# dohlee/rosettafold-pytorch

Hardware: AMD Instinct MI355X
Metric: residues/sec forward (L=256, N=128) (higher is better)
Workload: dtype bf16; 1 GPU; BASELINE.json configs[1]: bsz=4/GPU, n_seq=128, L=256, d_msa=384, d_pair=288, 8+5 blocks, 4 encoder layers, random-init weights; global_batch=4, parallelism=batch-sharded x1 (replicated weights), launch=one hipGraph replay per step (validation + input copy outside the graph)

## Files before the change

rosettafold-pytorch_amd/csrc/favor.hip:

```cpp
#include <type_traits>

#include "common.h"

#define FV_DH 64
#define FV_M 266
#define FV_MT 17
#define FV_MPAD 288
#define FV_CTX_LD 592
#define FV_DT 5
#define FV_DROWS 80

struct FavorAttnP {
  const h16_t* qkv;
  const h16_t* pc;
  h16_t* out;
  int64_t x_b, x_o, x_s;
  int64_t x_h;
  int64_t o_b, o_o, o_s;
  int q_off, k_off, v_off;
  int n_o, n_h, nitems;
  int nchunks;
  int dbg;
  float eps;
  float ctx_scale;
  int seq_len;
};

#ifdef RF_H16_IS_F16
#define FV_CS(x) ((x) * p.ctx_scale)
#else
#define FV_CS(x) (x)
#endif

typedef __attribute__((ext_vector_type(4))) short s16x4;

__device__ __forceinline__ int swz_off(int row, int chunk) { return row * 128 + ((chunk ^ (row & 7)) << 4); }

template <bool TAIL = false>
__device__ __forceinline__ void fv_load_tile(char* smem, int lds_off, const h16_t* g, int64_t stride, int nrows,
                                             int wave, int lane, int nvalid = 0) {
  const int ninstr = nrows * 8 / 64;
  for (int it = wave; it < ninstr; it += 4) {
    const int slot = it * 64 + lane;
    const int row = slot >> 3;
    const int clog = (slot & 7) ^ (row & 7);
    const int srow = TAIL ? (row < nvalid ? row : nvalid - 1) : row;
    rf_glds16(g + (int64_t)srow * stride + clog * 8, smem + lds_off + it * 1024);
  }
}

__device__ __forceinline__ float rbf(float x) { return h2f(f2h(x)); }

__device__ __forceinline__ float fv_mfma_done(float acc_reg) {
  asm volatile("s_nop 7\n\ts_nop 3" : "+v"(acc_reg));
  return acc_reg;
}

union Frag {
  h16x8 v;
  unsigned u[4];
  uint2 h[2];
};

template <int LS, bool SOFTMAX, bool TAIL>
__global__ __launch_bounds__(256, 1) void favor_attention_kernel(const FavorAttnP p) {
  constexpr int ST = LS / 64;
  constexpr int NSB = LS / 32;
  constexpr int PC_OFF = 0;
  constexpr int K_OFF = FV_MPAD * 128;
  constexpr int V_OFF = K_OFF + LS * 128;
  constexpr int CTX_OFF = V_OFF + LS * 128;
  constexpr int DIAG_OFF = CTX_OFF + FV_DROWS * FV_CTX_LD;
  constexpr int RED_OFF = DIAG_OFF + LS * 4;
  extern __shared__ __attribute__((aligned(16))) char smem[];
  const int tid = threadIdx.x, lane = tid & 63;
  const int wave = __builtin_amdgcn_readfirstlane(tid >> 6) & 3;
  const int fr = lane & 15, fq = lane >> 4;
  const int nm = wave == 0 ? 5 : 4;
  const int m0t = wave == 0 ? 0 : 5 + 4 * (wave - 1);
  const f32x4 epsv = {p.eps, p.eps, p.eps, p.eps};
  Frag ones;
#pragma unroll
  for (int k = 0; k < 4; ++k) ones.u[k] = fr == 0 ? RF_H16_ONE2 : 0u;

  fv_load_tile(smem, PC_OFF, p.pc, FV_DH, FV_MPAD, wave, lane);
  for (int i = tid; i < FV_DROWS * FV_CTX_LD / 4; i += 256) ((unsigned*)(smem + CTX_OFF))[i] = 0u;

  auto item_base = [&](int item, int64_t& xb, int64_t& ob) {
    const int h = item % p.n_h;
    const int t = item / p.n_h;
    const int o = t % p.n_o, b = t / p.n_o;
    xb = (int64_t)b * p.x_b + (int64_t)o * p.x_o + (int64_t)h * p.x_h;
    ob = (int64_t)b * p.o_b + (int64_t)o * p.o_o + h * FV_DH;
  };

  const int nch = p.nchunks;
  const int nv = TAIL ? p.seq_len : 0;
  int item = blockIdx.x;
  if (item < p.nitems) {
    int64_t xb, ob;
    item_base(item, xb, ob);
    fv_load_tile<TAIL>(smem, K_OFF, p.qkv + xb + p.k_off, p.x_s, LS, wave, lane, nv);
    fv_load_tile<TAIL>(smem, V_OFF, p.qkv + xb + p.v_off, p.x_s, LS, wave, lane, nv);
  }
  bool first = true;
  for (; item < p.nitems; item += gridDim.x) {
    int64_t xb, ob;
    item_base(item, xb, ob);
    if (first || TAIL)
      asm volatile("s_waitcnt vmcnt(0)" ::: "memory");
    else
      asm volatile("s_waitcnt vmcnt(%0)" ::"n"(ST * 4) : "memory");
    first = false;
    __syncthreads();
    h16x8 qf[ST][2];
    auto load_q = [&](int chunk) {
#pragma unroll
      for (int t = 0; t < ST; ++t) {
        int s = chunk * LS + (wave * ST + t) * 16 + fr;
        if (TAIL) s = s < nv ? s : nv - 1;
        const h16_t* qrow = p.qkv + xb + p.q_off + (int64_t)s * p.x_s;
#pragma unroll
        for (int kk = 0; kk < 2; ++kk) qf[t][kk] = *(const h16x8*)(qrow + (kk * 4 + fq) * 8);
      }
    };
    load_q(0);

    float gmax = 0.f;
    if constexpr (SOFTMAX) {
      for (int s = tid; s < LS; s += 256) {
        float a = 0.f;
#pragma unroll
        for (int c = 0; c < 8; ++c) {
          const h16x8 x = *(const h16x8*)(smem + K_OFF + s * 128 + c * 16);
#pragma unroll
          for (int e = 0; e < 8; ++e) {
            const float f = h2f((h16_t)x[e]);
            a = fmaf(f, f, a);
          }
        }
        ((float*)(smem + DIAG_OFF))[s] = a * (0.0625f * 1.4426950408889634f);
      }
    }

    h16x8 pf[5][2];
#pragma unroll
    for (int j = 0; j < 5; ++j)
#pragma unroll
      for (int kk = 0; kk < 2; ++kk)
        if (j < nm) pf[j][kk] = *(const h16x8*)(smem + PC_OFF + swz_off((m0t + j) * 16 + fr, kk * 4 + fq));

    if constexpr (SOFTMAX) {
      float mx = -INFINITY;
      const int nsb0 = TAIL ? (nv + 31) >> 5 : NSB;
      for (int u = 0; u < nsb0; ++u) {
        h16x8 kf[2][2];
#pragma unroll
        for (int t = 0; t < 2; ++t)
#pragma unroll
          for (int kk = 0; kk < 2; ++kk)
            kf[t][kk] = *(const h16x8*)(smem + K_OFF + swz_off((2 * u + t) * 16 + fr, kk * 4 + fq));
#pragma unroll
        for (int j = 0; j < 5; ++j) {
          if (j < nm) {
            const bool valid = (m0t + j) * 16 + fr < FV_M;
#pragma unroll
            for (int t = 0; t < 2; ++t) {
              f32x4 a = {0.f, 0.f, 0.f, 0.f};
              a = rf_mfma16(kf[t][0], pf[j][0], a, 0, 0, 0);
              a = rf_mfma16(kf[t][1], pf[j][1], a, 0, 0, 0);
              if (valid) mx = fmaxf(mx, fmaxf(fmaxf(a[0], a[1]), fmaxf(a[2], a[3])));
            }
          }
        }
      }
      mx = wave_max(mx);
      if (lane == 0) ((float*)(smem + RED_OFF))[wave] = mx;
      __syncthreads();
      const float* red = (const float*)(smem + RED_OFF);
      gmax = fmaxf(fmaxf(red[0], red[1]), fmaxf(red[2], red[3]));
    }

    f32x4 ctx[5][FV_DT];
#pragma unroll
    for (int j = 0; j < 5; ++j)
#pragma unroll
      for (int i = 0; i < FV_DT; ++i) ctx[j][i] = (f32x4){0.f, 0.f, 0.f, 0.f};
    for (int ck = 0; ck < nch; ++ck) {
    const int rem = TAIL ? nv - ck * LS : LS;
    if (ck > 0) {
      __syncthreads();
      fv_load_tile<TAIL>(smem, K_OFF, p.qkv + xb + p.k_off + (int64_t)ck * LS * p.x_s, p.x_s, LS, wave, lane, rem);
      fv_load_tile<TAIL>(smem, V_OFF, p.qkv + xb + p.v_off + (int64_t)ck * LS * p.x_s, p.x_s, LS, wave, lane, rem);
      asm volatile("s_waitcnt vmcnt(0)" ::: "memory");
      __syncthreads();
    }
    const int nsb = TAIL ? (rem < LS ? (rem + 31) >> 5 : NSB) : NSB;
    for (int u = 0; u < nsb; ++u) {
      h16x8 kf[2][2];
#pragma unroll
      for (int t = 0; t < 2; ++t)
#pragma unroll
        for (int kk = 0; kk < 2; ++kk)
          kf[t][kk] = *(const h16x8*)(smem + K_OFF + swz_off((2 * u + t) * 16 + fr, kk * 4 + fq));
      Frag vf[4];
      {
        const int p4 = fr & 3;
#pragma unroll
        for (int i = 0; i < 4; ++i) {
#pragma unroll
          for (int half = 0; half < 2; ++half) {
            const int row = u * 32 + half * 16 + 4 * fq + (fr >> 2);
            const int off = V_OFF + swz_off(row, i * 2 + (p4 >> 1)) + (p4 & 1) * 8;
            const s16x4 r = __builtin_amdgcn_ds_read_tr16_b64_v4i16((__attribute__((address_space(3))) s16x4*)(smem + off));
            vf[i].h[half] = __builtin_bit_cast(uint2, r);
          }
        }
      }
      f32x4 init[2] = {epsv, epsv};
      if constexpr (SOFTMAX) {
#pragma unroll
        for (int t = 0; t < 2; ++t) {
          const float4 d4 = *(const float4*)(smem + DIAG_OFF + ((2 * u + t) * 16 + 4 * fq) * 4);
          init[t] = (f32x4){-(d4.x + gmax), -(d4.y + gmax), -(d4.z + gmax), -(d4.w + gmax)};
        }
      }
#pragma unroll
      for (int j = 0; j < 5; ++j) {
        if (j < nm) {
          f32x4 a[2];
#pragma unroll
          for (int t = 0; t < 2; ++t) {
            a[t] = rf_mfma16(kf[t][0], pf[j][0], init[t], 0, 0, 0);
            a[t] = rf_mfma16(kf[t][1], pf[j][1], a[t], 0, 0, 0);
          }
          float f[2][4];
#pragma unroll
          for (int t = 0; t < 2; ++t)
#pragma unroll
            for (int r = 0; r < 4; ++r) {
              if constexpr (SOFTMAX)
                f[t][r] = __builtin_amdgcn_exp2f(a[t][r]) + p.eps;
              else
                f[t][r] = fmaxf(a[t][r], p.eps);
            }
          if ((m0t + j) == FV_MT - 1 && fr >= FV_M - 16 * (FV_MT - 1)) {
#pragma unroll
            for (int t = 0; t < 2; ++t)
#pragma unroll
              for (int r = 0; r < 4; ++r) f[t][r] = 0.f;
          }
          if constexpr (TAIL) {
            if ((u + 1) * 32 > rem) {
#pragma unroll
              for (int t = 0; t < 2; ++t)
#pragma unroll
                for (int r = 0; r < 4; ++r) f[t][r] = (2 * u + t) * 16 + 4 * fq + r < rem ? f[t][r] : 0.f;
            }
          }
          Frag kfr;
          kfr.u[0] = rf_pack2_h16(f[0][0], f[0][1]);
          kfr.u[1] = rf_pack2_h16(f[0][2], f[0][3]);
          kfr.u[2] = rf_pack2_h16(f[1][0], f[1][1]);
          kfr.u[3] = rf_pack2_h16(f[1][2], f[1][3]);
#pragma unroll
          for (int i = 0; i < 4; ++i)
            ctx[j][i] = rf_mfma16(kfr.v, vf[i].v, ctx[j][i], 0, 0, 0);
          ctx[j][4] = rf_mfma16(kfr.v, ones.v, ctx[j][4], 0, 0, 0);
        }
      }
    }
    }
#pragma unroll
    for (int j = 0; j < 5; ++j) {
      if (j < nm) {
#pragma unroll
        for (int i = 0; i < FV_DT; ++i) {
          uint2 w;
          w.x = rf_pack2_h16(FV_CS(ctx[j][i][0]), FV_CS(ctx[j][i][1]));
          w.y = rf_pack2_h16(FV_CS(ctx[j][i][2]), FV_CS(ctx[j][i][3]));
          *(uint2*)(smem + CTX_OFF + (i * 16 + fr) * FV_CTX_LD + ((m0t + j) * 16 + 4 * fq) * 2) = w;
        }
      }
    }
    __syncthreads();

    asm volatile("s_waitcnt vmcnt(0)" ::: "memory");
    {
      const int nxt = item + gridDim.x;
      if (nxt < p.nitems) {
        int64_t xb2, ob2;
        item_base(nxt, xb2, ob2);
        fv_load_tile<TAIL>(smem, K_OFF, p.qkv + xb2 + p.k_off, p.x_s, LS, wave, lane, nv);
        fv_load_tile<TAIL>(smem, V_OFF, p.qkv + xb2 + p.v_off, p.x_s, LS, wave, lane, nv);
      }
    }

    f32x4 qinit[ST];
#pragma unroll
    for (int t = 0; t < ST; ++t) qinit[t] = epsv;
    if constexpr (SOFTMAX) {
      float dq[ST], rmax[ST];
#pragma unroll
      for (int t = 0; t < ST; ++t) {
        float a = 0.f;
#pragma unroll
        for (int kk = 0; kk < 2; ++kk)
#pragma unroll
          for (int e = 0; e < 8; ++e) {
            const float f = h2f((h16_t)qf[t][kk][e]);
            a = fmaf(f, f, a);
          }
        a += __shfl_xor(a, 16, 64);
        a += __shfl_xor(a, 32, 64);
        dq[t] = a * (0.0625f * 1.4426950408889634f);
        rmax[t] = -INFINITY;
      }
      for (int j = 0; j < FV_MT; ++j) {
        h16x8 pfr[2];
#pragma unroll
        for (int kk = 0; kk < 2; ++kk) pfr[kk] = *(const h16x8*)(smem + PC_OFF + swz_off(j * 16 + fr, kk * 4 + fq));
#pragma unroll
        for (int t = 0; t < ST; ++t) {
          f32x4 a = {0.f, 0.f, 0.f, 0.f};
          a = rf_mfma16(pfr[0], qf[t][0], a, 0, 0, 0);
          a = rf_mfma16(pfr[1], qf[t][1], a, 0, 0, 0);
#pragma unroll
          for (int r = 0; r < 4; ++r)
            if (j * 16 + 4 * fq + r < FV_M) rmax[t] = fmaxf(rmax[t], a[r]);
        }
      }
#pragma unroll
      for (int t = 0; t < ST; ++t) {
        rmax[t] = fmaxf(rmax[t], __shfl_xor(rmax[t], 16, 64));
        rmax[t] = fmaxf(rmax[t], __shfl_xor(rmax[t], 32, 64));
        const float off = -(dq[t] + rmax[t]);
        qinit[t] = (f32x4){off, off, off, off};
      }
    }
    for (int qc = 0; qc < nch; ++qc) {
    if (TAIL && qc * LS + wave * ST * 16 >= nv) continue;
    if (qc > 0) load_q(qc);
    f32x4 num[FV_DT][ST];
#pragma unroll
    for (int t = 0; t < ST; ++t)
#pragma unroll
      for (int i = 0; i < FV_DT; ++i) num[i][t] = (f32x4){0.f, 0.f, 0.f, 0.f};
    auto mblock = [&](int u, auto last_tag) {
      constexpr bool LAST = decltype(last_tag)::value;
      float f[2][ST][4];
#pragma unroll
      for (int jj = 0; jj < 2; ++jj) {
        if (LAST && jj == 1) {
#pragma unroll
          for (int t = 0; t < ST; ++t)
#pragma unroll
            for (int r = 0; r < 4; ++r) f[jj][t][r] = 0.f;
        } else {
          const int j = 2 * u + jj;
          h16x8 pfr[2];
#pragma unroll
          for (int kk = 0; kk < 2; ++kk) pfr[kk] = *(const h16x8*)(smem + PC_OFF + swz_off(j * 16 + fr, kk * 4 + fq));
#pragma unroll
          for (int t = 0; t < ST; ++t) {
            f32x4 a = rf_mfma16(pfr[0], qf[t][0], qinit[t], 0, 0, 0);
            a = rf_mfma16(pfr[1], qf[t][1], a, 0, 0, 0);
#pragma unroll
            for (int r = 0; r < 4; ++r) {
              float x;
              if constexpr (SOFTMAX)
                x = __builtin_amdgcn_exp2f(a[r]) + p.eps;
              else
                x = fmaxf(a[r], p.eps);
              if (LAST && 4 * fq + r >= FV_M - 16 * (FV_MT - 1)) x = 0.f;
              f[jj][t][r] = x;
            }
          }
        }
      }
      Frag cf[FV_DT];
#pragma unroll
      for (int i = 0; i < FV_DT; ++i) {
        const char* base = smem + CTX_OFF + (i * 16 + fr) * FV_CTX_LD + (32 * u + 4 * fq) * 2;
        cf[i].h[0] = *(const uint2*)base;
        cf[i].h[1] = *(const uint2*)(base + 32);
      }
#pragma unroll
      for (int t = 0; t < ST; ++t) {
        Frag qfr;
        qfr.u[0] = rf_pack2_h16(f[0][t][0], f[0][t][1]);
        qfr.u[1] = rf_pack2_h16(f[0][t][2], f[0][t][3]);
        qfr.u[2] = rf_pack2_h16(f[1][t][0], f[1][t][1]);
        qfr.u[3] = rf_pack2_h16(f[1][t][2], f[1][t][3]);
#pragma unroll
        for (int i = 0; i < FV_DT; ++i)
          num[i][t] = rf_mfma16(cf[i].v, qfr.v, num[i][t], 0, 0, 0);
      }
    };
    for (int u = 0; u < (FV_MT - 1) / 2; ++u) mblock(u, std::false_type{});
    mblock((FV_MT - 1) / 2, std::true_type{});
#pragma unroll
    for (int t = 0; t < ST; ++t) {
      const float dn = __shfl(fv_mfma_done(num[4][t][0]), fr, 64);
      const float inv = 1.f / dn;
      const int s = qc * LS + (wave * ST + t) * 16 + fr;
      h16_t* orow = p.out + ob + (int64_t)s * p.o_s;
#pragma unroll
      for (int i = 0; i < 4; ++i) {
        uint2 w;
        w.x = rf_pack2_h16(num[i][t][0] * inv, num[i][t][1] * inv);
        w.y = rf_pack2_h16(num[i][t][2] * inv, num[i][t][3] * inv);
        if (!TAIL || s < nv) *(uint2*)(orow + i * 16 + 4 * fq) = w;
      }
    }
    }
  }
}

#pragma clang diagnostic ignored "-Winline-asm"
__device__ __forceinline__ void fv_glds_asm(const void* src, unsigned lds_addr) {
  asm volatile("s_mov_b32 m0, %0\n\ts_nop 0\n\tglobal_load_lds_dwordx4 %1, off" ::"s"(lds_addr), "v"(src) : "memory", "m0");
}

__device__ __forceinline__ void fv_lds_barrier() {
  asm volatile("s_waitcnt lgkmcnt(0)" ::: "memory");
  __builtin_amdgcn_s_barrier();
  asm volatile("" ::: "memory");
}

__device__ unsigned long long g_fv_cycles[8];
#define FV_STAMP(slot)                                                   \
  if (prof) {                                                            \
    const unsigned long long now = __builtin_readcyclecounter();         \
    acc_cyc[slot] += now - t_last;                                       \
    t_last = now;                                                        \
  }

template <int LS, bool SOFTMAX, bool TAIL>
__global__ __launch_bounds__(512, 1) void favor_attention_kernel8(const FavorAttnP p) {
  constexpr int NSB = LS / 32;
  constexpr int NJ = 3;
  constexpr int STB = LS >= 128 ? LS / 128 : 1;
  constexpr int NWB = LS / (16 * STB);
  constexpr int PC_OFF = 0;
  constexpr int K_OFF = FV_MPAD * 128;
  constexpr int V_OFF = K_OFF + LS * 128;
  constexpr int CTX_OFF = V_OFF + LS * 128;
  constexpr int DIAG_OFF = CTX_OFF + FV_DROWS * FV_CTX_LD;
  constexpr int RED_OFF = DIAG_OFF + LS * 4;
  extern __shared__ __attribute__((aligned(16))) char smem[];
  const int tid = threadIdx.x, lane = tid & 63;
  const int wave = __builtin_amdgcn_readfirstlane(tid >> 6) & 7;
  const int fr = lane & 15, fq = lane >> 4;
  const int nm = wave == 0 ? 3 : 2;
  const int m0t = wave == 0 ? 0 : 1 + 2 * wave;
  const f32x4 epsv = {p.eps, p.eps, p.eps, p.eps};
  Frag ones;
#pragma unroll
  for (int k = 0; k < 4; ++k) ones.u[k] = fr == 0 ? RF_H16_ONE2 : 0u;

  const unsigned lds_base = (unsigned)(uintptr_t)(__attribute__((address_space(3))) char*)smem;
  auto load_tile8 = [&](int lds_off, const h16_t* gp, int64_t stride, auto nrows_tag, int nvalid = 0) {
    constexpr int NI = decltype(nrows_tag)::value * 8 / 64;
    int ln = lane;
    asm volatile("" : "+v"(ln));
    const int dma_row = ln >> 3;
    const int dma_col = ((ln & 7) ^ dma_row) * 8;
    const h16_t* g0 = gp + (int64_t)dma_row * stride + dma_col;
#pragma unroll
    for (int k = 0; k < (NI + 7) / 8; ++k) {
      const int it = wave + 8 * k;
      if (NI % 8 == 0 || it < NI) {
        const unsigned dst = __builtin_amdgcn_readfirstlane(lds_base + lds_off + it * 1024);
        if (TAIL && nvalid > 0) {
          const int row = dma_row + 8 * it;
          fv_glds_asm(gp + (int64_t)(row < nvalid ? row : nvalid - 1) * stride + dma_col, dst);
        } else {
          fv_glds_asm(g0 + (int64_t)(8 * it) * stride, dst);
        }
      }
    }
  };
  constexpr std::integral_constant<int, LS> LS_TAG{};
  load_tile8(PC_OFF, p.pc, FV_DH, std::integral_constant<int, FV_MPAD>{});
  for (int i = tid; i < FV_DROWS * FV_CTX_LD / 4; i += 512) ((unsigned*)(smem + CTX_OFF))[i] = 0u;

  auto item_base = [&](int item, int64_t& xb, int64_t& ob) {
    const int h = item % p.n_h;
    const int t = item / p.n_h;
    const int o = t % p.n_o, b = t / p.n_o;
    xb = (int64_t)b * p.x_b + (int64_t)o * p.x_o + (int64_t)h * p.x_h;
    ob = (int64_t)b * p.o_b + (int64_t)o * p.o_o + h * FV_DH;
  };
  auto ctx_col = [](int tile, int q4) { return ((tile >> 1) * 32 + 8 * q4 + 4 * (tile & 1)) * 2; };
  const int nch = SOFTMAX ? 1 : p.nchunks;
  const int nv = TAIL ? p.seq_len : 0;
  int item = blockIdx.x;
  if (item < p.nitems) {
    int64_t xb, ob;
    item_base(item, xb, ob);
    load_tile8(K_OFF, p.qkv + xb + p.k_off, p.x_s, LS_TAG, nv);
    load_tile8(V_OFF, p.qkv + xb + p.v_off, p.x_s, LS_TAG, nv);
  }
  bool first = true;
  const bool prof = (RF_DBG(p.dbg) & 8) && wave == ((RF_DBG(p.dbg) >> 4) & 7);
  unsigned long long acc_cyc[7] = {0, 0, 0, 0, 0, 0, 0};
  unsigned long long t_last = prof ? __builtin_readcyclecounter() : 0;
  for (; item < p.nitems; item += gridDim.x) {
    int64_t xb, ob;
    item_base(item, xb, ob);
    asm volatile("" : "+v"(xb), "+v"(ob));
    if (prof) {
      t_last = __builtin_readcyclecounter();
      acc_cyc[6] += 1;
    }
    if (first || wave >= NWB || TAIL)
      asm volatile("s_waitcnt vmcnt(0)" ::: "memory");
    else
      asm volatile("s_waitcnt vmcnt(%0)" ::"n"(STB * 4) : "memory");
    first = false;
    fv_lds_barrier();
    FV_STAMP(0)
    h16x8 pf[NJ][2];
    {
      int frP = fr, fqP = fq;
      asm volatile("" : "+v"(frP), "+v"(fqP));
#pragma unroll
      for (int j = 0; j < NJ; ++j)
#pragma unroll
        for (int kk = 0; kk < 2; ++kk)
          pf[j][kk] = *(const h16x8*)(smem + PC_OFF + m0t * 2048 + swz_off(frP, kk * 4 + fqP) + (j < nm ? j : 0) * 2048);
    }
    h16x8 qf[STB][2];
    auto load_q = [&](int chunk) {
      int frq = fr, fqq = fq;
      asm volatile("" : "+v"(frq), "+v"(fqq));
      if (wave < NWB) {
#pragma unroll
        for (int t = 0; t < STB; ++t) {
          int s = chunk * LS + (wave * STB + t) * 16 + frq;
          if (TAIL) s = s < nv ? s : nv - 1;
          const h16_t* qrow = p.qkv + xb + p.q_off + (int64_t)s * p.x_s;
#pragma unroll
          for (int kk = 0; kk < 2; ++kk) qf[t][kk] = *(const h16x8*)(qrow + (kk * 4 + fqq) * 8);
        }
      }
    };
    load_q(0);

    float gmax = 0.f;
    if constexpr (SOFTMAX) {
      int frS = fr, fqS = fq;
      asm volatile("" : "+v"(frS), "+v"(fqS));
      for (int s = tid; s < LS; s += 512) {
        float a = 0.f;
#pragma unroll
        for (int c = 0; c < 8; ++c) {
          const h16x8 x = *(const h16x8*)(smem + K_OFF + s * 128 + c * 16);
#pragma unroll
          for (int e = 0; e < 8; ++e) {
            const float f = h2f((h16_t)x[e]);
            a = fmaf(f, f, a);
          }
        }
        ((float*)(smem + DIAG_OFF))[s] = a * (0.0625f * 1.4426950408889634f);
      }
      float mx = -INFINITY;
      const int nsb0 = TAIL ? (nv + 31) >> 5 : NSB;
      for (int u = 0; u < nsb0; ++u) {
        h16x8 kf[2][2];
#pragma unroll
        for (int t = 0; t < 2; ++t)
#pragma unroll
          for (int kk = 0; kk < 2; ++kk)
            kf[t][kk] = *(const h16x8*)(smem + K_OFF + swz_off((2 * u + t) * 16 + frS, kk * 4 + fqS));
#pragma unroll
        for (int j = 0; j < NJ; ++j) {
          if (j < nm) {
            const h16x8* pfj = pf[j];
            const bool valid = (m0t + j) != FV_MT - 1 || frS < FV_M - 16 * (FV_MT - 1);
#pragma unroll
            for (int t = 0; t < 2; ++t) {
              f32x4 a = {0.f, 0.f, 0.f, 0.f};
              a = rf_mfma16(kf[t][0], pfj[0], a, 0, 0, 0);
              a = rf_mfma16(kf[t][1], pfj[1], a, 0, 0, 0);
              if (valid) mx = fmaxf(mx, fmaxf(fmaxf(a[0], a[1]), fmaxf(a[2], a[3])));
            }
          }
        }
      }
      mx = wave_max(mx);
      if (lane == 0) ((float*)(smem + RED_OFF))[wave] = mx;
      fv_lds_barrier();
      const float* red = (const float*)(smem + RED_OFF);
      gmax = fmaxf(fmaxf(fmaxf(red[0], red[1]), fmaxf(red[2], red[3])), fmaxf(fmaxf(red[4], red[5]), fmaxf(red[6], red[7])));
    }

    f32x4 ctx[NJ][FV_DT];
#pragma unroll
    for (int j = 0; j < NJ; ++j)
#pragma unroll
      for (int i = 0; i < FV_DT; ++i) ctx[j][i] = (f32x4){0.f, 0.f, 0.f, 0.f};
    for (int ck = 0; ck < nch; ++ck) {
      const int rem = TAIL ? nv - ck * LS : LS;
      if (ck > 0) {
        __syncthreads();
        load_tile8(K_OFF, p.qkv + xb + p.k_off + (int64_t)ck * LS * p.x_s, p.x_s, LS_TAG, rem);
        load_tile8(V_OFF, p.qkv + xb + p.v_off + (int64_t)ck * LS * p.x_s, p.x_s, LS_TAG, rem);
        asm volatile("s_waitcnt vmcnt(0)" ::: "memory");
        __syncthreads();
      }
      const int nsb = TAIL ? (rem < LS ? (rem + 31) >> 5 : NSB) : NSB;
      h16x8 kf[2][2];
      Frag vf[4];
      auto load_sblock = [&](int u, h16x8 (&kfo)[2][2], Frag (&vfo)[4]) {
#pragma unroll
        for (int t = 0; t < 2; ++t)
#pragma unroll
          for (int kk = 0; kk < 2; ++kk)
            kfo[t][kk] = *(const h16x8*)(smem + K_OFF + swz_off((2 * u + t) * 16 + fr, kk * 4 + fq));
        const int p4 = fr & 3;
#pragma unroll
        for (int i = 0; i < 4; ++i) {
#pragma unroll
          for (int half = 0; half < 2; ++half) {
            const int row = u * 32 + half * 16 + 4 * fq + (fr >> 2);
            const int off = V_OFF + swz_off(row, i * 2 + (p4 >> 1)) + (p4 & 1) * 8;
            const s16x4 r = __builtin_amdgcn_ds_read_tr16_b64_v4i16((__attribute__((address_space(3))) s16x4*)(smem + off));
            vfo[i].h[half] = __builtin_bit_cast(uint2, r);
          }
        }
      };
      load_sblock(0, kf, vf);
      for (int u = 0; u < ((RF_DBG(p.dbg) & 1) ? 0 : nsb); ++u) {
        h16x8 kfn[2][2];
        Frag vfn[4];
        load_sblock(u + 1 < nsb ? u + 1 : u, kfn, vfn);
        f32x4 init[2] = {epsv, epsv};
        if constexpr (SOFTMAX) {
#pragma unroll
          for (int t = 0; t < 2; ++t) {
            const float4 d4 = *(const float4*)(smem + DIAG_OFF + ((2 * u + t) * 16 + 4 * fq) * 4);
            init[t] = (f32x4){-(d4.x + gmax), -(d4.y + gmax), -(d4.z + gmax), -(d4.w + gmax)};
          }
        }
#pragma unroll
        for (int j = 0; j < NJ; ++j) {
          if (j < nm) {
            const h16x8* pfj = pf[j];
            f32x4 a[2];
#pragma unroll
            for (int t = 0; t < 2; ++t) {
              a[t] = rf_mfma16(kf[t][0], pfj[0], init[t], 0, 0, 0);
              a[t] = rf_mfma16(kf[t][1], pfj[1], a[t], 0, 0, 0);
            }
            float f[2][4];
#pragma unroll
            for (int t = 0; t < 2; ++t)
#pragma unroll
              for (int r = 0; r < 4; ++r) {
                if constexpr (SOFTMAX)
                  f[t][r] = __builtin_amdgcn_exp2f(a[t][r]) + p.eps;
                else
                  f[t][r] = fmaxf(a[t][r], p.eps);
              }
            if ((m0t + j) == FV_MT - 1 && fr >= FV_M - 16 * (FV_MT - 1)) {
#pragma unroll
              for (int t = 0; t < 2; ++t)
#pragma unroll
                for (int r = 0; r < 4; ++r) f[t][r] = 0.f;
            }
            if constexpr (TAIL) {
              if ((u + 1) * 32 > rem) {
#pragma unroll
                for (int t = 0; t < 2; ++t)
#pragma unroll
                  for (int r = 0; r < 4; ++r) f[t][r] = (2 * u + t) * 16 + 4 * fq + r < rem ? f[t][r] : 0.f;
              }
            }
            Frag kfr;
            kfr.u[0] = rf_pack2_h16(f[0][0], f[0][1]);
            kfr.u[1] = rf_pack2_h16(f[0][2], f[0][3]);
            kfr.u[2] = rf_pack2_h16(f[1][0], f[1][1]);
            kfr.u[3] = rf_pack2_h16(f[1][2], f[1][3]);
#pragma unroll
            for (int i = 0; i < 4; ++i)
              ctx[j][i] = rf_mfma16(kfr.v, vf[i].v, ctx[j][i], 0, 0, 0);
            ctx[j][4] = rf_mfma16(kfr.v, ones.v, ctx[j][4], 0, 0, 0);
          }
        }
#pragma unroll
        for (int t = 0; t < 2; ++t)
#pragma unroll
          for (int kk = 0; kk < 2; ++kk) kf[t][kk] = kfn[t][kk];
#pragma unroll
        for (int i = 0; i < 4; ++i) vf[i] = vfn[i];
      }
    }
    FV_STAMP(1)
#pragma unroll
    for (int j = 0; j < NJ; ++j)
      if (j < nm) {
#pragma unroll
        for (int i = 0; i < FV_DT; ++i) {
          uint2 w;
          w.x = rf_pack2_h16(FV_CS(ctx[j][i][0]), FV_CS(ctx[j][i][1]));
          w.y = rf_pack2_h16(FV_CS(ctx[j][i][2]), FV_CS(ctx[j][i][3]));
          *(uint2*)(smem + CTX_OFF + (i * 16 + fr) * FV_CTX_LD + ctx_col(m0t + j, fq)) = w;
        }
      }
    fv_lds_barrier();
    FV_STAMP(2)
    asm volatile("s_waitcnt vmcnt(0)" ::: "memory");
#pragma unroll
    for (int t = 0; t < STB; ++t) {
      asm volatile("" : "+v"(qf[t][0]), "+v"(qf[t][1]));
    }
    {
      const int nxt = item + gridDim.x;
      if (nxt < p.nitems) {
        int64_t xb2, ob2;
        item_base(nxt, xb2, ob2);
        load_tile8(K_OFF, p.qkv + xb2 + p.k_off, p.x_s, LS_TAG, nv);
        load_tile8(V_OFF, p.qkv + xb2 + p.v_off, p.x_s, LS_TAG, nv);
      }
    }
    FV_STAMP(3)
    for (int qc = 0; qc < nch; ++qc) {
      if (qc > 0) {
        load_q(qc);
        asm volatile("s_waitcnt vmcnt(0)" ::: "memory");
#pragma unroll
        for (int t = 0; t < STB; ++t) {
          asm volatile("" : "+v"(qf[t][0]), "+v"(qf[t][1]));
        }
      }
      if (wave < NWB && (!TAIL || qc * LS + wave * STB * 16 < nv)) {
        f32x4 qinit[STB];
#pragma unroll
        for (int t = 0; t < STB; ++t) qinit[t] = epsv;
        if constexpr (SOFTMAX) {
          float dq[STB], rmax[STB];
#pragma unroll
          for (int t = 0; t < STB; ++t) {
            float a = 0.f;
#pragma unroll
            for (int kk = 0; kk < 2; ++kk)
#pragma unroll
              for (int e = 0; e < 8; ++e) {
                const float f = h2f((h16_t)qf[t][kk][e]);
                a = fmaf(f, f, a);
              }
            a += __shfl_xor(a, 16, 64);
            a += __shfl_xor(a, 32, 64);
            dq[t] = a * (0.0625f * 1.4426950408889634f);
            rmax[t] = -INFINITY;
          }
          for (int j = 0; j < FV_MT; ++j) {
            h16x8 pfr[2];
#pragma unroll
            for (int kk = 0; kk < 2; ++kk) pfr[kk] = *(const h16x8*)(smem + PC_OFF + swz_off(j * 16 + fr, kk * 4 + fq));
#pragma unroll
            for (int t = 0; t < STB; ++t) {
              f32x4 a = {0.f, 0.f, 0.f, 0.f};
              a = rf_mfma16(pfr[0], qf[t][0], a, 0, 0, 0);
              a = rf_mfma16(pfr[1], qf[t][1], a, 0, 0, 0);
#pragma unroll
              for (int r = 0; r < 4; ++r)
                if (j * 16 + 4 * fq + r < FV_M) rmax[t] = fmaxf(rmax[t], a[r]);
            }
          }
#pragma unroll
          for (int t = 0; t < STB; ++t) {
            rmax[t] = fmaxf(rmax[t], __shfl_xor(rmax[t], 16, 64));
            rmax[t] = fmaxf(rmax[t], __shfl_xor(rmax[t], 32, 64));
            const float off = -(dq[t] + rmax[t]);
            qinit[t] = (f32x4){off, off, off, off};
          }
        }
        f32x4 num[FV_DT][STB];
#pragma unroll
        for (int t = 0; t < STB; ++t)
#pragma unroll
          for (int i = 0; i < FV_DT; ++i) num[i][t] = (f32x4){0.f, 0.f, 0.f, 0.f};
        auto mblock = [&](int u, auto last_tag) {
          constexpr bool LAST = decltype(last_tag)::value;
          float f[2][STB][4];
#pragma unroll
          for (int jj = 0; jj < 2; ++jj) {
            if (LAST && jj == 1) {
#pragma unroll
              for (int t = 0; t < STB; ++t)
#pragma unroll
                for (int r = 0; r < 4; ++r) f[jj][t][r] = 0.f;
            } else {
              const int j = 2 * u + jj;
              h16x8 pfr[2];
#pragma unroll
              for (int kk = 0; kk < 2; ++kk) pfr[kk] = *(const h16x8*)(smem + PC_OFF + swz_off(j * 16 + fr, kk * 4 + fq));
#pragma unroll
              for (int t = 0; t < STB; ++t) {
                f32x4 a = rf_mfma16(pfr[0], qf[t][0], qinit[t], 0, 0, 0);
                a = rf_mfma16(pfr[1], qf[t][1], a, 0, 0, 0);
#pragma unroll
                for (int r = 0; r < 4; ++r) {
                  float x;
                  if constexpr (SOFTMAX)
                    x = __builtin_amdgcn_exp2f(a[r]) + p.eps;
                  else
                    x = fmaxf(a[r], p.eps);
                  if (LAST && 4 * fq + r >= FV_M - 16 * (FV_MT - 1)) x = 0.f;
                  f[jj][t][r] = x;
                }
              }
            }
          }
          Frag cf[FV_DT];
#pragma unroll
          for (int i = 0; i < FV_DT; ++i)
            cf[i].v = *(const h16x8*)(smem + CTX_OFF + (i * 16 + fr) * FV_CTX_LD + (32 * u + 8 * fq) * 2);
#pragma unroll
          for (int t = 0; t < STB; ++t) {
            Frag qfr;
            qfr.u[0] = rf_pack2_h16(f[0][t][0], f[0][t][1]);
            qfr.u[1] = rf_pack2_h16(f[0][t][2], f[0][t][3]);
            qfr.u[2] = rf_pack2_h16(f[1][t][0], f[1][t][1]);
            qfr.u[3] = rf_pack2_h16(f[1][t][2], f[1][t][3]);
#pragma unroll
            for (int i = 0; i < FV_DT; ++i)
              num[i][t] = rf_mfma16(cf[i].v, qfr.v, num[i][t], 0, 0, 0);
          }
        };
        for (int u = 0; u < ((RF_DBG(p.dbg) & 2) ? 0 : (FV_MT - 1) / 2); ++u) mblock(u, std::false_type{});
        mblock((FV_MT - 1) / 2, std::true_type{});
        FV_STAMP(4)
#pragma unroll
        for (int t = 0; t < STB; ++t) {
          const float dn = __shfl(fv_mfma_done(num[4][t][0]), fr, 64);
          const float inv = 1.f / dn;
          const int s = qc * LS + (wave * STB + t) * 16 + fr;
          h16_t* orow = p.out + ob + (int64_t)s * p.o_s;
#pragma unroll
          for (int i = 0; i < 4; ++i) {
            uint2 w;
            w.x = rf_pack2_h16(num[i][t][0] * inv, num[i][t][1] * inv);
            w.y = rf_pack2_h16(num[i][t][2] * inv, num[i][t][3] * inv);
            if (!TAIL || s < nv) *(uint2*)(orow + i * 16 + 4 * fq) = w;
          }
        }
      }
    }
    FV_STAMP(5)
  }
  if (prof && lane == 0) {
#pragma unroll
    for (int i = 0; i < 7; ++i) atomicAdd(&g_fv_cycles[i], acc_cyc[i]);
  }
}

extern "C" int rf_favor_phase_cycles(unsigned long long* out7, int reset) {
  unsigned long long z[8] = {0, 0, 0, 0, 0, 0, 0, 0};
  if (out7 && hipMemcpyFromSymbol(out7, HIP_SYMBOL(g_fv_cycles), 7 * sizeof(unsigned long long)) != hipSuccess) return 1000 + (int)hipGetLastError();
  if (reset && hipMemcpyToSymbol(HIP_SYMBOL(g_fv_cycles), z, sizeof(z)) != hipSuccess) return 1000 + (int)hipGetLastError();
  return 0;
}

template <int LS, bool SM, bool TAIL>
static int launch_favor(const FavorAttnP& p, hipStream_t s) {
  const size_t lds = (size_t)FV_MPAD * 128 + 2 * (size_t)LS * 128 + (size_t)FV_DROWS * FV_CTX_LD + LS * 4 + 64;
  const int ncu = rf_num_cus() > 0 ? rf_num_cus() : 256;
  const int grid = p.nitems < ncu ? p.nitems : ncu;
  static const bool force4 = getenv("RF_FAVOR4") != nullptr;
  constexpr bool only4 = SM && LS > 128;
  if (only4 || force4) {
    auto k = favor_attention_kernel<LS, SM, TAIL>;
    if (const int e = rf_enable_big_lds<favor_attention_kernel<LS, SM, TAIL>>()) return e;
    hipLaunchKernelGGL(k, dim3(grid), dim3(256), lds, s, p);
  } else if constexpr (!only4) {
    auto k = favor_attention_kernel8<LS, SM, TAIL>;
    if (const int e = rf_enable_big_lds<favor_attention_kernel8<LS, SM, TAIL>>()) return e;
    hipLaunchKernelGGL(k, dim3(grid), dim3(512), lds, s, p);
  }
  return rf_launch_status();
}

extern "C" int rf_favor_attention(const void* qkv, const void* pc, void* out, const int64_t x_strides[4],
                                  const int64_t o_strides[3], int q_off, int k_off, int v_off, int n_b, int n_o,
                                  int n_h, int seq_len, int dim_head, int n_features, int softmax_kernel, float eps,
                                  void* stream) {
  if (dim_head != FV_DH || n_features != FV_M) return RF_EINVAL;
  if (seq_len < 1) return RF_EINVAL;
  int nchunks = 1, ls = seq_len <= 64 ? 64 : seq_len <= 128 ? 128 : 256;
  if (seq_len > 256) {
    if (softmax_kernel) return RF_EINVAL;
    nchunks = (seq_len + 255) / 256;
  }
  const bool tail = seq_len != nchunks * ls;
  if (((uintptr_t)qkv % 16) || ((uintptr_t)pc % 16) || ((uintptr_t)out % 8)) return RF_EALIGN;
  for (int i = 0; i < 3; ++i)
    if (x_strides[i] % 8 || o_strides[i] % 4) return RF_EALIGN;
  if (x_strides[3] % 8) return RF_EALIGN;
  if (q_off % 8 || k_off % 8 || v_off % 8) return RF_EALIGN;
  FavorAttnP p;
  p.qkv = (const h16_t*)qkv;
  p.pc = (const h16_t*)pc;
  p.out = (h16_t*)out;
  p.x_b = x_strides[0]; p.x_o = x_strides[1]; p.x_s = x_strides[2]; p.x_h = x_strides[3];
  p.o_b = o_strides[0]; p.o_o = o_strides[1]; p.o_s = o_strides[2];
  p.q_off = q_off; p.k_off = k_off; p.v_off = v_off;
  p.n_o = n_o; p.n_h = n_h;
  p.nitems = n_b * n_o * n_h;
  p.eps = eps;
  p.nchunks = nchunks;
  p.seq_len = seq_len;
  p.ctx_scale = 1.0f;
#ifdef RF_H16_IS_F16
  for (int n = 1; n < seq_len; n <<= 1) p.ctx_scale *= 0.5f;
#endif
  static int dbg = 0;
  static const int dbg_rc = rf_dbg_env("RF_FAVOR_DBG", &dbg);
  if (dbg_rc) return dbg_rc;
  p.dbg = dbg;
  hipStream_t s = (hipStream_t)stream;
#define FV_LAUNCH(LS_) \
  (tail ? (softmax_kernel ? launch_favor<LS_, true, true>(p, s) : launch_favor<LS_, false, true>(p, s)) \
        : (softmax_kernel ? launch_favor<LS_, true, false>(p, s) : launch_favor<LS_, false, false>(p, s)))
  if (ls == 256) return FV_LAUNCH(256);
  if (ls == 128) return FV_LAUNCH(128);
  return FV_LAUNCH(64);
#undef FV_LAUNCH
}
```

Baseline: 3126 residues/s.

## Cache softmax FAVOR feature logits in registers to skip recomputing MFMAs

In the softmax FAVOR attention path, the key-side and query-side projection logits computed during the max pass are now kept in registers (kl, ql). The second pass reuses them instead of re-running the MFMAs and reloading the projection and key fragments from LDS. Loops are fully unrolled so the register arrays stay statically indexed. Tail masking moves to a packed bitmask on the bf16 fragments. The cost is much higher register pressure, which may cause spills, plus a static_assert limiting the softmax form to LS<=128.

```diff
diff --git a/rosettafold-pytorch_amd/csrc/favor.hip b/rosettafold-pytorch_amd/csrc/favor.hip
--- a/rosettafold-pytorch_amd/csrc/favor.hip
+++ b/rosettafold-pytorch_amd/csrc/favor.hip
@@ -442,6 +442,7 @@
   constexpr int NJ = 3;
   constexpr int STB = LS >= 128 ? LS / 128 : 1;
   constexpr int NWB = LS / (16 * STB);
+  static_assert(!SOFTMAX || LS <= 128, "the softmax form keeps LS / 16 key-logit tiles per feature tile and STB = 1 query tiles");
   constexpr int PC_OFF = 0;
   constexpr int K_OFF = FV_MPAD * 128;
   constexpr int V_OFF = K_OFF + LS * 128;
@@ -461,6 +462,7 @@
 
   const unsigned lds_base = (unsigned)(uintptr_t)(__attribute__((address_space(3))) char*)smem;
   auto load_tile8 = [&](int lds_off, const h16_t* gp, int64_t stride, auto nrows_tag, int nvalid = 0) {
+    constexpr bool CLAMP = TAIL && decltype(nrows_tag)::value == LS;
     constexpr int NI = decltype(nrows_tag)::value * 8 / 64;
     int ln = lane;
     asm volatile("" : "+v"(ln));
@@ -472,7 +474,7 @@
       const int it = wave + 8 * k;
       if (NI % 8 == 0 || it < NI) {
         const unsigned dst = __builtin_amdgcn_readfirstlane(lds_base + lds_off + it * 1024);
-        if (TAIL && nvalid > 0) {
+        if constexpr (CLAMP) {
           const int row = dma_row + 8 * it;
           fv_glds_asm(gp + (int64_t)(row < nvalid ? row : nvalid - 1) * stride + dma_col, dst);
         } else {
@@ -514,10 +516,11 @@
       t_last = __builtin_readcyclecounter();
       acc_cyc[6] += 1;
     }
-    if (first || wave >= NWB || TAIL)
+    if (first || wave >= NWB || TAIL) {
       asm volatile("s_waitcnt vmcnt(0)" ::: "memory");
-    else
+    } else {
       asm volatile("s_waitcnt vmcnt(%0)" ::"n"(STB * 4) : "memory");
+    }
     first = false;
     fv_lds_barrier();
     FV_STAMP(0)
@@ -549,6 +552,7 @@
     load_q(0);
 
     float gmax = 0.f;
+    f32x4 kl[SOFTMAX ? NJ : 1][SOFTMAX ? 2 * NSB : 1];
     if constexpr (SOFTMAX) {
       int frS = fr, fqS = fq;
       asm volatile("" : "+v"(frS), "+v"(fqS));
@@ -566,25 +570,30 @@
         ((float*)(smem + DIAG_OFF))[s] = a * (0.0625f * 1.4426950408889634f);
       }
       float mx = -INFINITY;
-      const int nsb0 = TAIL ? (nv + 31) >> 5 : NSB;
-      for (int u = 0; u < nsb0; ++u) {
-        h16x8 kf[2][2];
-#pragma unroll
-        for (int t = 0; t < 2; ++t)
-#pragma unroll
-          for (int kk = 0; kk < 2; ++kk)
-            kf[t][kk] = *(const h16x8*)(smem + K_OFF + swz_off((2 * u + t) * 16 + frS, kk * 4 + fqS));
-#pragma unroll
-        for (int j = 0; j < NJ; ++j) {
-          if (j < nm) {
-            const h16x8* pfj = pf[j];
-            const bool valid = (m0t + j) != FV_MT - 1 || frS < FV_M - 16 * (FV_MT - 1);
-#pragma unroll
-            for (int t = 0; t < 2; ++t) {
-              f32x4 a = {0.f, 0.f, 0.f, 0.f};
-              a = rf_mfma16(kf[t][0], pfj[0], a, 0, 0, 0);
-              a = rf_mfma16(kf[t][1], pfj[1], a, 0, 0, 0);
-              if (valid) mx = fmaxf(mx, fmaxf(fmaxf(a[0], a[1]), fmaxf(a[2], a[3])));
+      int nsb0 = TAIL ? (nv + 31) >> 5 : NSB;
+      if constexpr (TAIL) asm volatile("" : "+s"(nsb0));
+#pragma unroll
+      for (int u = 0; u < NSB; ++u) {
+        if (!TAIL || u < nsb0) {
+          h16x8 kf[2][2];
+#pragma unroll
+          for (int t = 0; t < 2; ++t)
+#pragma unroll
+            for (int kk = 0; kk < 2; ++kk)
+              kf[t][kk] = *(const h16x8*)(smem + K_OFF + swz_off((2 * u + t) * 16 + frS, kk * 4 + fqS));
+#pragma unroll
+          for (int j = 0; j < NJ; ++j) {
+            if (j < nm) {
+              const h16x8* pfj = pf[j];
+              const bool valid = (m0t + j) != FV_MT - 1 || frS < FV_M - 16 * (FV_MT - 1);
+#pragma unroll
+              for (int t = 0; t < 2; ++t) {
+                f32x4 a = {0.f, 0.f, 0.f, 0.f};
+                a = rf_mfma16(kf[t][0], pfj[0], a, 0, 0, 0);
+                a = rf_mfma16(kf[t][1], pfj[1], a, 0, 0, 0);
+                kl[j][2 * u + t] = a;
+                if (valid) mx = fmaxf(mx, fmaxf(fmaxf(a[0], a[1]), fmaxf(a[2], a[3])));
+              }
             }
           }
         }
@@ -596,6 +605,8 @@
       gmax = fmaxf(fmaxf(fmaxf(red[0], red[1]), fmaxf(red[2], red[3])), fmaxf(fmaxf(red[4], red[5]), fmaxf(red[6], red[7])));
     }
 
+    int frA = fr, fqA = fq;
+    if constexpr (SOFTMAX) asm volatile("" : "+v"(frA), "+v"(fqA));
     f32x4 ctx[NJ][FV_DT];
 #pragma unroll
     for (int j = 0; j < NJ; ++j)
@@ -610,21 +621,24 @@
         asm volatile("s_waitcnt vmcnt(0)" ::: "memory");
         __syncthreads();
       }
-      const int nsb = TAIL ? (rem < LS ? (rem + 31) >> 5 : NSB) : NSB;
+      int nsb = TAIL ? (rem < LS ? (rem + 31) >> 5 : NSB) : NSB;
+      if constexpr (TAIL && SOFTMAX) asm volatile("" : "+s"(nsb));
       h16x8 kf[2][2];
       Frag vf[4];
       auto load_sblock = [&](int u, h16x8 (&kfo)[2][2], Frag (&vfo)[4]) {
-#pragma unroll
-        for (int t = 0; t < 2; ++t)
-#pragma unroll
-          for (int kk = 0; kk < 2; ++kk)
-            kfo[t][kk] = *(const h16x8*)(smem + K_OFF + swz_off((2 * u + t) * 16 + fr, kk * 4 + fq));
-        const int p4 = fr & 3;
+        if constexpr (!SOFTMAX) {
+#pragma unroll
+          for (int t = 0; t < 2; ++t)
+#pragma unroll
+            for (int kk = 0; kk < 2; ++kk)
+              kfo[t][kk] = *(const h16x8*)(smem + K_OFF + swz_off((2 * u + t) * 16 + frA, kk * 4 + fqA));
+        }
+        const int p4 = frA & 3;
 #pragma unroll
         for (int i = 0; i < 4; ++i) {
 #pragma unroll
           for (int half = 0; half < 2; ++half) {
-            const int row = u * 32 + half * 16 + 4 * fq + (fr >> 2);
+            const int row = u * 32 + half * 16 + 4 * fqA + (frA >> 2);
             const int off = V_OFF + swz_off(row, i * 2 + (p4 >> 1)) + (p4 & 1) * 8;
             const s16x4 r = __builtin_amdgcn_ds_read_tr16_b64_v4i16((__attribute__((address_space(3))) s16x4*)(smem + off));
             vfo[i].h[half] = __builtin_bit_cast(uint2, r);
@@ -632,27 +646,42 @@
         }
       };
       load_sblock(0, kf, vf);
-      for (int u = 0; u < ((RF_DBG(p.dbg) & 1) ? 0 : nsb); ++u) {
+      auto sblock = [&](const int u) {
         h16x8 kfn[2][2];
         Frag vfn[4];
-        load_sblock(u + 1 < nsb ? u + 1 : u, kfn, vfn);
+        load_sblock(SOFTMAX ? (u + 1 < NSB ? u + 1 : u) : (u + 1 < nsb ? u + 1 : u), kfn, vfn);
         f32x4 init[2] = {epsv, epsv};
         if constexpr (SOFTMAX) {
 #pragma unroll
           for (int t = 0; t < 2; ++t) {
-            const float4 d4 = *(const float4*)(smem + DIAG_OFF + ((2 * u + t) * 16 + 4 * fq) * 4);
+            const float4 d4 = *(const float4*)(smem + DIAG_OFF + ((2 * u + t) * 16 + 4 * fqA) * 4);
             init[t] = (f32x4){-(d4.x + gmax), -(d4.y + gmax), -(d4.z + gmax), -(d4.w + gmax)};
+          }
+        }
+        unsigned mk[4] = {~0u, ~0u, ~0u, ~0u};
+        if constexpr (SOFTMAX && TAIL) {
+          int left = rem - 4 * fqA;
+          asm volatile("" : "+v"(left));
+#pragma unroll
+          for (int i = 0; i < 4; ++i) {
+            const int r0 = (2 * u + (i >> 1)) * 16 + 2 * (i & 1);
+            mk[i] = ((unsigned)((r0 - left) >> 31) & 0xFFFFu) | ((unsigned)((r0 + 1 - left) >> 31) & 0xFFFF0000u);
           }
         }
 #pragma unroll
         for (int j = 0; j < NJ; ++j) {
           if (j < nm) {
-            const h16x8* pfj = pf[j];
             f32x4 a[2];
-#pragma unroll
-            for (int t = 0; t < 2; ++t) {
-              a[t] = rf_mfma16(kf[t][0], pfj[0], init[t], 0, 0, 0);
-              a[t] = rf_mfma16(kf[t][1], pfj[1], a[t], 0, 0, 0);
+            if constexpr (SOFTMAX) {
+#pragma unroll
+              for (int t = 0; t < 2; ++t) a[t] = kl[j][2 * u + t] + init[t];
+            } else {
+              const h16x8* pfj = pf[j];
+#pragma unroll
+              for (int t = 0; t < 2; ++t) {
+                a[t] = rf_mfma16(kf[t][0], pfj[0], init[t], 0, 0, 0);
+                a[t] = rf_mfma16(kf[t][1], pfj[1], a[t], 0, 0, 0);
+              }
             }
             float f[2][4];
 #pragma unroll
@@ -664,18 +693,18 @@
                 else
                   f[t][r] = fmaxf(a[t][r], p.eps);
               }
-            if ((m0t + j) == FV_MT - 1 && fr >= FV_M - 16 * (FV_MT - 1)) {
+            if ((m0t + j) == FV_MT - 1 && frA >= FV_M - 16 * (FV_MT - 1)) {
 #pragma unroll
               for (int t = 0; t < 2; ++t)
 #pragma unroll
                 for (int r = 0; r < 4; ++r) f[t][r] = 0.f;
             }
-            if constexpr (TAIL) {
+            if constexpr (TAIL && !SOFTMAX) {
               if ((u + 1) * 32 > rem) {
 #pragma unroll
                 for (int t = 0; t < 2; ++t)
 #pragma unroll
-                  for (int r = 0; r < 4; ++r) f[t][r] = (2 * u + t) * 16 + 4 * fq + r < rem ? f[t][r] : 0.f;
+                  for (int r = 0; r < 4; ++r) f[t][r] = (2 * u + t) * 16 + 4 * fqA + r < rem ? f[t][r] : 0.f;
               }
             }
             Frag kfr;
@@ -683,18 +712,32 @@
             kfr.u[1] = rf_pack2_h16(f[0][2], f[0][3]);
             kfr.u[2] = rf_pack2_h16(f[1][0], f[1][1]);
             kfr.u[3] = rf_pack2_h16(f[1][2], f[1][3]);
+            if constexpr (SOFTMAX && TAIL) {
+#pragma unroll
+              for (int i = 0; i < 4; ++i) kfr.u[i] &= mk[i];
+            }
 #pragma unroll
             for (int i = 0; i < 4; ++i)
               ctx[j][i] = rf_mfma16(kfr.v, vf[i].v, ctx[j][i], 0, 0, 0);
             ctx[j][4] = rf_mfma16(kfr.v, ones.v, ctx[j][4], 0, 0, 0);
           }
         }
-#pragma unroll
-        for (int t = 0; t < 2; ++t)
-#pragma unroll
-          for (int kk = 0; kk < 2; ++kk) kf[t][kk] = kfn[t][kk];
+        if constexpr (!SOFTMAX) {
+#pragma unroll
+          for (int t = 0; t < 2; ++t)
+#pragma unroll
+            for (int kk = 0; kk < 2; ++kk) kf[t][kk] = kfn[t][kk];
+        }
 #pragma unroll
         for (int i = 0; i < 4; ++i) vf[i] = vfn[i];
+      };
+      const bool run_a = !(RF_DBG(p.dbg) & 1);
+      if constexpr (SOFTMAX) {
+#pragma unroll
+        for (int u = 0; u < NSB; ++u)
+          if (run_a && (!TAIL || u < nsb)) sblock(u);
+      } else {
+        for (int u = 0; u < (run_a ? nsb : 0); ++u) sblock(u);
       }
     }
     FV_STAMP(1)
@@ -706,7 +749,7 @@
           uint2 w;
           w.x = rf_pack2_h16(FV_CS(ctx[j][i][0]), FV_CS(ctx[j][i][1]));
           w.y = rf_pack2_h16(FV_CS(ctx[j][i][2]), FV_CS(ctx[j][i][3]));
-          *(uint2*)(smem + CTX_OFF + (i * 16 + fr) * FV_CTX_LD + ctx_col(m0t + j, fq)) = w;
+          *(uint2*)(smem + CTX_OFF + (i * 16 + frA) * FV_CTX_LD + ctx_col(m0t + j, fqA)) = w;
         }
       }
     fv_lds_barrier();
@@ -736,9 +779,12 @@
         }
       }
       if (wave < NWB && (!TAIL || qc * LS + wave * STB * 16 < nv)) {
+        int frB = fr, fqB = fq;
+        if constexpr (SOFTMAX) asm volatile("" : "+v"(frB), "+v"(fqB));
         f32x4 qinit[STB];
 #pragma unroll
         for (int t = 0; t < STB; ++t) qinit[t] = epsv;
+        f32x4 ql[SOFTMAX ? FV_MT : 1][STB];
         if constexpr (SOFTMAX) {
           float dq[STB], rmax[STB];
 #pragma unroll
@@ -756,20 +802,29 @@
             dq[t] = a * (0.0625f * 1.4426950408889634f);
             rmax[t] = -INFINITY;
           }
-          for (int j = 0; j < FV_MT; ++j) {
+          auto maxtile = [&](const int j, auto last_tag) {
+            constexpr bool LASTT = decltype(last_tag)::value;
             h16x8 pfr[2];
 #pragma unroll
-            for (int kk = 0; kk < 2; ++kk) pfr[kk] = *(const h16x8*)(smem + PC_OFF + swz_off(j * 16 + fr, kk * 4 + fq));
+            for (int kk = 0; kk < 2; ++kk) pfr[kk] = *(const h16x8*)(smem + PC_OFF + swz_off(j * 16 + frB, kk * 4 + fqB));
 #pragma unroll
             for (int t = 0; t < STB; ++t) {
               f32x4 a = {0.f, 0.f, 0.f, 0.f};
               a = rf_mfma16(pfr[0], qf[t][0], a, 0, 0, 0);
               a = rf_mfma16(pfr[1], qf[t][1], a, 0, 0, 0);
-#pragma unroll
-              for (int r = 0; r < 4; ++r)
-                if (j * 16 + 4 * fq + r < FV_M) rmax[t] = fmaxf(rmax[t], a[r]);
+              ql[j][t] = a;
+              if constexpr (LASTT) {
+#pragma unroll
+                for (int r = 0; r < 4; ++r)
+                  if (4 * fqB + r < FV_M - 16 * (FV_MT - 1)) rmax[t] = fmaxf(rmax[t], a[r]);
+              } else {
+                rmax[t] = fmaxf(rmax[t], fmaxf(fmaxf(a[0], a[1]), fmaxf(a[2], a[3])));
+              }
             }
-          }
+          };
+#pragma unroll
+          for (int j = 0; j < FV_MT - 1; ++j) maxtile(j, std::false_type{});
+          maxtile(FV_MT - 1, std::true_type{});
 #pragma unroll
           for (int t = 0; t < STB; ++t) {
             rmax[t] = fmaxf(rmax[t], __shfl_xor(rmax[t], 16, 64));
@@ -796,12 +851,19 @@
             } else {
               const int j = 2 * u + jj;
               h16x8 pfr[2];
-#pragma unroll
-              for (int kk = 0; kk < 2; ++kk) pfr[kk] = *(const h16x8*)(smem + PC_OFF + swz_off(j * 16 + fr, kk * 4 + fq));
+              if constexpr (!SOFTMAX) {
+#pragma unroll
+                for (int kk = 0; kk < 2; ++kk) pfr[kk] = *(const h16x8*)(smem + PC_OFF + swz_off(j * 16 + frB, kk * 4 + fqB));
+              }
 #pragma unroll
               for (int t = 0; t < STB; ++t) {
-                f32x4 a = rf_mfma16(pfr[0], qf[t][0], qinit[t], 0, 0, 0);
-                a = rf_mfma16(pfr[1], qf[t][1], a, 0, 0, 0);
+                f32x4 a;
+                if constexpr (SOFTMAX) {
+                  a = ql[j][t] + qinit[t];
+                } else {
+                  a = rf_mfma16(pfr[0], qf[t][0], qinit[t], 0, 0, 0);
+                  a = rf_mfma16(pfr[1], qf[t][1], a, 0, 0, 0);
+                }
 #pragma unroll
                 for (int r = 0; r < 4; ++r) {
                   float x;
@@ -809,7 +871,7 @@
                     x = __builtin_amdgcn_exp2f(a[r]) + p.eps;
                   else
                     x = fmaxf(a[r], p.eps);
-                  if (LAST && 4 * fq + r >= FV_M - 16 * (FV_MT - 1)) x = 0.f;
+                  if (LAST && 4 * fqB + r >= FV_M - 16 * (FV_MT - 1)) x = 0.f;
                   f[jj][t][r] = x;
                 }
               }
@@ -818,7 +880,7 @@
           Frag cf[FV_DT];
 #pragma unroll
           for (int i = 0; i < FV_DT; ++i)
-            cf[i].v = *(const h16x8*)(smem + CTX_OFF + (i * 16 + fr) * FV_CTX_LD + (32 * u + 8 * fq) * 2);
+            cf[i].v = *(const h16x8*)(smem + CTX_OFF + (i * 16 + frB) * FV_CTX_LD + (32 * u + 8 * fqB) * 2);
 #pragma unroll
           for (int t = 0; t < STB; ++t) {
             Frag qfr;
@@ -831,21 +893,28 @@
               num[i][t] = rf_mfma16(cf[i].v, qfr.v, num[i][t], 0, 0, 0);
           }
         };
-        for (int u = 0; u < ((RF_DBG(p.dbg) & 2) ? 0 : (FV_MT - 1) / 2); ++u) mblock(u, std::false_type{});
+        const bool run_b = !(RF_DBG(p.dbg) & 2);
+        if constexpr (SOFTMAX) {
+#pragma unroll
+          for (int u = 0; u < (FV_MT - 1) / 2; ++u)
+            if (run_b) mblock(u, std::false_type{});
+        } else {
+          for (int u = 0; u < (run_b ? (FV_MT - 1) / 2 : 0); ++u) mblock(u, std::false_type{});
+        }
         mblock((FV_MT - 1) / 2, std::true_type{});
         FV_STAMP(4)
 #pragma unroll
         for (int t = 0; t < STB; ++t) {
-          const float dn = __shfl(fv_mfma_done(num[4][t][0]), fr, 64);
+          const float dn = __shfl(fv_mfma_done(num[4][t][0]), frB, 64);
           const float inv = 1.f / dn;
-          const int s = qc * LS + (wave * STB + t) * 16 + fr;
+          const int s = qc * LS + (wave * STB + t) * 16 + frB;
           h16_t* orow = p.out + ob + (int64_t)s * p.o_s;
 #pragma unroll
           for (int i = 0; i < 4; ++i) {
             uint2 w;
             w.x = rf_pack2_h16(num[i][t][0] * inv, num[i][t][1] * inv);
             w.y = rf_pack2_h16(num[i][t][2] * inv, num[i][t][3] * inv);
-            if (!TAIL || s < nv) *(uint2*)(orow + i * 16 + 4 * fq) = w;
+            if (!TAIL || s < nv) *(uint2*)(orow + i * 16 + 4 * fqB) = w;
           }
         }
       }
```

After: 3180 residues/s, median of 6. +1.7%, better.
